# snayfach/MicrobeCensus

Hardware: AMD Instinct MI355X
Metric: reads/sec searched vs marker DB + AGS abs-error, 150 bp @ 1/2/4/8 GPU (higher is better)
Workload: dtype u8/int32

## Files before the change

microbecensus_amd/csrc/k_gapped.h:

```cpp
#pragma once
#include "mc_hip_common.h"

struct McFlankOut { int16_t gain, c1, c2, ident, steps, runs, gapcols, over; };

struct McFlank { int qoff, doff, st, n1, n2; };
__device__ __forceinline__ bool mc_flank_of(const McGapTask &g, int qlen, int dlen, int side, McFlank &f)
{
    if (side == 0) {
        const int qend = g.qfwd + g.qp + g.L, dend = g.qfwd + g.dp + g.L;
        f.qoff = qend; f.doff = dend; f.st = 1; f.n1 = qlen - qend; f.n2 = dlen - dend;
    } else {
        const int qleft = g.qp - g.qbwd, dleft = g.dp - g.qbwd;
        f.qoff = qleft - 1; f.doff = dleft - 1; f.st = -1; f.n1 = qleft; f.n2 = dleft;
    }
    return f.n1 > 2 && f.n2 > 2;
}

__device__ __forceinline__ bool mc_gap_same_segment(const McGapTask &a, const McGapTask &b)
{
    return a.read == b.read && a.sidx == b.sidx && (a.chrono >> 25) == (b.chrono >> 25) && a.qp - a.qbwd == b.qp - b.qbwd && a.dp - a.qbwd == b.dp - b.qbwd &&
           a.qp + a.L + a.qfwd == b.qp + b.L + b.qfwd;
}

__device__ __forceinline__ uint32_t mc_block_alloc_n(uint32_t *counter, uint32_t n)
{
    __shared__ uint32_t wcnt[4], wbase[4];
    const int lane = mc_lane(), wv = threadIdx.x >> 6;
    uint32_t incl = n;
    for (int d = 1; d < 64; d <<= 1) { const uint32_t y = __shfl_up(incl, d); if (lane >= d) incl += y; }
    if (lane == 63) wcnt[wv] = incl;
    __syncthreads();
    if (threadIdx.x == 0) {
        const uint32_t c0 = wcnt[0], c1 = wcnt[1], c2 = wcnt[2], c3 = wcnt[3], tot = c0 + c1 + c2 + c3;
        const uint32_t b = tot ? atomicAdd(counter, tot) : 0u;
        wbase[0] = b; wbase[1] = b + c0; wbase[2] = b + c0 + c1; wbase[3] = b + c0 + c1 + c2;
    }
    __syncthreads();
    const uint32_t r = wbase[wv] + incl - n;
    __syncthreads();
    return r;
}

__global__ void __launch_bounds__(256) k_gap_dedupe(McIndex X, int L, const McGapTask *__restrict__ gaps, uint32_t ngaps, unsigned long long *tab, uint32_t mask, uint32_t *leader,
                                                    uint32_t *key, uint32_t *item, uint32_t *counters)
{
    const uint32_t p = blockIdx.x * 256 + threadIdx.x;
    uint32_t n = 0;
    McFlank fr, fl;
    bool hr = false, hl = false;
    if (p < ngaps && gaps[p].read == MC_TASK_NONE) leader[p] = p;
    else if (p < ngaps) {
        const McGapTask g = gaps[p];
        unsigned long long h = ((unsigned long long)g.read << 32) ^ ((unsigned long long)g.sidx << 12) ^ (unsigned long long)(g.chrono >> 25);
        h ^= ((unsigned long long)(uint16_t)(g.qp - g.qbwd) << 48) ^ ((unsigned long long)(uint16_t)(g.dp - g.qbwd) << 20) ^ ((unsigned long long)(uint16_t)(g.qp + g.L + g.qfwd) << 3);
        h *= 0x9E3779B97F4A7C15ull; h ^= h >> 29; h *= 0xBF58476D1CE4E5B9ull; h ^= h >> 32;
        const unsigned long long mine = (h & ~0x7FFFFFFull) | (unsigned long long)(p + 1);
        uint32_t slot = (uint32_t)h & mask, who = p;
        bool lead = false;
        for (;;) {
            unsigned long long e = tab[slot];
            if (e == 0) e = atomicCAS(&tab[slot], 0ull, mine);
            if (e == 0) { lead = true; break; }
            if ((e & ~0x7FFFFFFull) == (mine & ~0x7FFFFFFull)) {
                const uint32_t q = (uint32_t)(e & 0x7FFFFFFull) - 1;
                if (mc_gap_same_segment(g, gaps[q])) { who = q; break; }
            }
            slot = (slot + 1) & mask;
        }
        leader[p] = who;
        if (lead) {
            const int frame = (int)(g.chrono >> 25), qlen = (L - frame % 3) / 3, dlen = (int)(X.off[g.sidx + 1] - X.off[g.sidx]);
            hr = mc_flank_of(g, qlen, dlen, 0, fr); hl = mc_flank_of(g, qlen, dlen, 1, fl);
            n = (hr ? 1u : 0u) + (hl ? 1u : 0u);
        }
    }
    uint32_t o = mc_block_alloc_n(&counters[C_ITEMS], n);
    if (hr) { key[o] = 1u + (uint32_t)fr.n1; item[o] = 2 * p; o++; }
    if (hl) { key[o] = 1u + (uint32_t)fl.n1; item[o] = 2 * p + 1; }
}

#define MC_GS_BINS 1024u
__global__ void __launch_bounds__(256) k_gap_sort_hist(const uint32_t *__restrict__ key, const uint32_t *__restrict__ n_p, uint32_t cap, uint32_t *hist)
{
    __shared__ uint32_t h[MC_GS_BINS];
    const uint32_t n = *n_p <= cap ? *n_p : 0u;
    for (uint32_t b = threadIdx.x; b < MC_GS_BINS; b += 256) h[b] = 0;
    __syncthreads();
    const uint32_t per = (n + gridDim.x - 1) / gridDim.x, lo = blockIdx.x * per, hi = lo + per < n ? lo + per : n;
    for (uint32_t i = lo + threadIdx.x; i < hi; i += 256) atomicAdd(&h[key[i] & (MC_GS_BINS - 1)], 1u);
    __syncthreads();
    for (uint32_t b = threadIdx.x; b < MC_GS_BINS; b += 256) if (h[b]) atomicAdd(&hist[b], h[b]);
}
__global__ void __launch_bounds__(1024) k_gap_sort_scan(uint32_t *hist)
{
    __shared__ uint32_t s[MC_GS_BINS];
    const uint32_t t = threadIdx.x, v = hist[MC_GS_BINS - 1 - t];
    s[t] = v;
    __syncthreads();
    for (uint32_t d = 1; d < MC_GS_BINS; d <<= 1) { const uint32_t y = t >= d ? s[t - d] : 0u; __syncthreads(); s[t] += y; __syncthreads(); }
    hist[MC_GS_BINS - 1 - t] = s[t] - v;
}
__global__ void __launch_bounds__(256) k_gap_sort_scatter(const uint32_t *__restrict__ key, const uint32_t *__restrict__ item, const uint32_t *__restrict__ n_p, uint32_t cap, uint32_t *base, uint32_t *out)
{
    __shared__ uint32_t h[MC_GS_BINS], at[MC_GS_BINS];
    const uint32_t n = *n_p <= cap ? *n_p : 0u;
    for (uint32_t b = threadIdx.x; b < MC_GS_BINS; b += 256) h[b] = 0;
    __syncthreads();
    const uint32_t per = (n + gridDim.x - 1) / gridDim.x, lo = blockIdx.x * per, hi = lo + per < n ? lo + per : n;
    for (uint32_t i = lo + threadIdx.x; i < hi; i += 256) atomicAdd(&h[key[i] & (MC_GS_BINS - 1)], 1u);
    __syncthreads();
    for (uint32_t b = threadIdx.x; b < MC_GS_BINS; b += 256) { const uint32_t c = h[b]; if (c) at[b] = atomicAdd(&base[b], c); h[b] = 0; }
    __syncthreads();
    for (uint32_t i = lo + threadIdx.x; i < hi; i += 256) { const uint32_t b = key[i] & (MC_GS_BINS - 1); out[at[b] + atomicAdd(&h[b], 1u)] = item[i]; }
}

__global__ void __launch_bounds__(256) k_gap_emit(const McTables *__restrict__ T, McIndex X, int L, const McGapTask *__restrict__ gaps, uint32_t ngaps, const uint32_t *__restrict__ leader,
                                                  const McFlankOut *__restrict__ fout, McHsp *hsps, uint32_t cap_hsps, uint32_t *counters, const McClassPars *__restrict__ P,
                                                  const int32_t *__restrict__ fam, uint8_t *cand, uint64_t *hkeys, uint8_t *low, uint64_t *hplace)
{
    const uint32_t p = blockIdx.x * 256 + threadIdx.x;
    bool keep = false;
    McHsp h;
    if (p < ngaps && gaps[p].read != MC_TASK_NONE) {
        const McGapTask g = gaps[p];
        const uint32_t ld = leader[p];
        const int frame = (int)(g.chrono >> 25), qlen = (L - frame % 3) / 3, dlen = (int)(X.off[g.sidx + 1] - X.off[g.sidx]);
        int score = g.score, nmatch = g.nmatch, qfwd = g.qfwd, dfwd = g.qfwd, qbwd = g.qbwd, dbwd = g.qbwd, alnlen = g.qfwd + g.L + g.qbwd, gapopens = 0, gaptotal = 0;
        McFlank f;
        if (mc_flank_of(g, qlen, dlen, 0, f)) {
            const McFlankOut R = fout[2 * (size_t)ld];
            if (R.gain > 0) { score += R.gain; nmatch += R.ident; qfwd += R.c1; dfwd += R.c2; alnlen += R.steps; gapopens += R.runs; gaptotal += R.gapcols; }
        }
        if (mc_flank_of(g, qlen, dlen, 1, f)) {
            const McFlankOut R = fout[2 * (size_t)ld + 1];
            if (R.gain > 0) { score += R.gain; nmatch += R.ident; qbwd += R.c1; dbwd += R.c2; alnlen += R.steps; gapopens += R.runs; gaptotal += R.gapcols; }
        }
        h.read = g.read; h.chrono = g.chrono;
        keep = mc_make_hsp(*T, L, frame, g, qfwd, dfwd, qbwd, dbwd, score, nmatch, alnlen, gapopens, gaptotal, &h);
        if (keep && cand && mc_hsp_can_classify(*T, *P, X, fam, h)) cand[h.read] = 1;
        if (keep && h.loge < T->loge_thr) low[h.read] = 1;
    }
    const uint32_t o = mc_block_alloc(&counters[C_HSPS], keep);
    if (keep) { if (o < cap_hsps) { hsps[o] = h; hkeys[o] = MC_HSP_KEY(h); hplace[o] = MC_HSP_PLACE(h); } else counters[C_OVERFLOW] = 2; }
}

#define MC_GAP_W 1200
#ifndef MC_GAP_WIN
#define MC_GAP_WIN 36
#endif
#ifndef MC_GAP_WIN2
#define MC_GAP_WIN2 64
#endif
static_assert(MC_GAP_WIN >= 16 && MC_GAP_WIN <= MC_GAP_WIN2, "row 0 of a flank has jEnd + 1 = 16 columns (xdrop_gapped 26.98: mc_gap_begin), and the second window is no narrower than the first");
#define MC_GAP_LANES2 64

__device__ __forceinline__ McFlankOut mc_flank_out(const McGapResult &R)
{
    McFlankOut o;
    o.gain = (int16_t)R.gain; o.c1 = (int16_t)R.c1; o.c2 = (int16_t)R.c2; o.ident = (int16_t)R.ident; o.steps = (int16_t)R.steps; o.runs = (int16_t)R.runs;
    o.gapcols = (int16_t)R.gapcols; o.over = (int16_t)R.overflow;
    return o;
}

__global__ void __launch_bounds__(128) k_gapped(const McTables *__restrict__ T, McIndex X, const uint8_t *__restrict__ frames, int FP, int L,
                                                const McGapTask *__restrict__ gaps, const uint32_t *__restrict__ list, const uint32_t *__restrict__ nitems_p, McFlankOut *fout,
                                                uint32_t *counters, McGapCell *ws, int cap)
{
    __shared__ McHot hot;
    const uint32_t nitems = *nitems_p;
    if (nitems == 0) return;
    mc_load_hot(&hot, T);
    __syncthreads();
    const uint32_t tid = blockIdx.x * blockDim.x + threadIdx.x, nthreads = gridDim.x * blockDim.x;
    McGapCell *C = ws + (size_t)tid * cap;
    for (uint32_t k0 = tid; k0 < nitems; k0 += nthreads) {
        const uint32_t it = list[k0];
        const McGapTask g = gaps[it >> 1];
        const int frame = (int)(g.chrono >> 25), qlen = (L - frame % 3) / 3;
        const uint32_t o0 = X.off[g.sidx];
        McFlank f;
        (void)mc_flank_of(g, qlen, (int)(X.off[g.sidx + 1] - o0), (int)(it & 1), f);
        const McGapResult R = mc_align_gapped(hot, frames + ((int64_t)g.read * 6 + frame) * FP + f.qoff, f.st, X.res + o0 + f.doff, f.st, f.n1, f.n2, C, cap);
        if (R.overflow) counters[C_OVERFLOW] = 5;
        fout[it] = mc_flank_out(R);
    }
}

#define MC_GAP_REFILL 8
template <int W>
struct McGapLds {
    uint2 *cell;
    uint32_t ovf;
    __device__ __forceinline__ void load(int c, int &H, int &D, uint32_t &PH, uint32_t &PD) const
    {
        const uint2 w = cell[c * 64];
        mc_gap_unpack(w.x, w.y, H, D, PH, PD);
    }
    __device__ __forceinline__ void store(int c, int H, int D, uint32_t PH, uint32_t PD)
    {
        uint2 w;
        ovf |= mc_gap_pack(H, D, PH, PD, w.x, w.y);
        cell[c * 64] = w;
    }
    __device__ __forceinline__ int loadH(int c) const { return (int)(cell[c * 64].x << 20) >> 20; }
};

template <int W, int LANES, int REFILL>
__global__ void __launch_bounds__(64) k_gapped_lds(const McTables *__restrict__ T, McIndex X, const uint8_t *__restrict__ frames, int FP, int L,
                                                   const McGapTask *__restrict__ gaps, const uint32_t *__restrict__ list, const uint32_t *__restrict__ nitems_p, McFlankOut *fout,
                                                   uint32_t *retry_count, uint32_t *retry, uint32_t *take)
{
    static_assert(REFILL >= 1 && REFILL <= LANES, "a refill is at most the lanes that take items");
    __shared__ McHot hot;
    __shared__ uint2 win[W * 64];
    const uint32_t nitems = *nitems_p;
    if (nitems == 0) return;
    mc_load_hot(&hot, T);
    __syncthreads();
    const int lane = threadIdx.x;
    McGapLds<W> ws; ws.cell = win + lane; ws.ovf = 0;
    const bool mine = lane < LANES;
    const uint32_t G = gridDim.x, w0 = blockIdx.x;
    constexpr uint32_t WS = (uint32_t)LANES;
    uint32_t wpos = w0 * WS < nitems ? w0 * WS : nitems, wend = wpos + WS < nitems ? wpos + WS : nitems;
    uint32_t pend = 0;
    bool asked = false, dry = false;
    const unsigned long long lt = (1ull << lane) - 1;
    bool active = false;
// ... 73 lines not shown
```

microbecensus_amd/csrc/mc_hip.hip:

```cpp
#include "mc_hip_common.h"
#include "k_translate_seg.h"
#include "k_enumerate.h"
#include "k_eval_seeds.h"
#include "k_gapped.h"
#include "k_order.h"
#include "k_finish.h"
#include "k_grid.h"
#include "k_simulate.h"
#include "k_community.h"
#include "k_varlen.h"
#include "k_classes.h"
#include "k_bootstrap.h"
#include "k_wfit.h"
#include "k_abundance.h"
#include "k_coverage.h"
#include "mc_pieces.h"
#include "mc_owned.h"

#include <map>

struct McCtx {
    McStream stream; hipStream_t side = nullptr, side2 = nullptr;
    McEvent ev[8], ev_fork, ev_join, ev_join2;
    int64_t cap_reads = 0; int pool_len = 0;
    uint32_t cap_tasks = 0, cap_gaps = 0, cap_hsps = 0, cap_rows = 0;
    McDev<uint8_t> d_frames_base; uint8_t *d_frames = nullptr;
    McDev<unsigned long long> d_stats;
    McDev<McSeedTask> d_tasks; McDev<McGapTask> d_gaps; McDev<McHsp> d_hsps, d_v, d_tmp;
    McDev<uint64_t> d_k64, d_hkeys, d_hplace, d_places; McDev<uint32_t> d_idx, d_idxo, d_heads, d_scan, d_gsz, d_nv, d_ghist;
    McDev<uint32_t> d_counters;
    McDev<McRow> d_rows; McDev<uint32_t> d_nrow, d_rowoff; McDev<McBestHit> d_best, d_bestof; McDev<uint8_t> d_low, d_cand;
    McDev<McGapCell> d_gws_full; McDev<uint32_t> d_retry, d_retry2; int gap_threads_full = 0;
    McDev<unsigned long long> d_gtab; uint32_t gtab_slots = 0; McDev<uint32_t> d_gleader; McDev<McFlankOut> d_fout;
    McPin<uint32_t> h_c; McPin<unsigned long long> h_stats; McPin<McBestHit> h_best; size_t h_best_cap = 0;
    const uint8_t *reads = nullptr; int64_t n = 0, first_read_id = 0;
    uint32_t ntasks = 0, ngaps = 0, gpad = 0, nh = 0, nh_all = 0, nheads = 0, nrows = 0, nbest = 0, nsegs = 0;
    bool busy = false;
};

struct mc_handle {
    McHostIndex H;
    std::vector<int32_t> fam;
    int nfam = 0, device = 0;
    McDev<uint8_t> d_res_base; uint8_t *d_res = nullptr; McDev<uint32_t> d_off, d_bstart, d_post; McDev<unsigned long long> d_post8; McDev<uint16_t> d_keys; McDev<int32_t> d_fam;
    McDev<McTables> d_T; McDev<McClassPars> d_P;
    McTables hT; McClassPars hP;
    int read_len = 0, FP = 0; bool run_set = false;
    McDev<uint32_t> d_bitmap;
    McDev<McBucketRec> d_rec;
    McDev<uint32_t> d_filt, d_wild, d_pair; McDev<uint64_t> d_segtab; McDev<unsigned long long> d_rt;
    bool fast_enum = false;
    bool count_traffic = false;
    int pipe_nout = 0;
    bool keep_rows = true;
    bool best_only = false;
    bool rows_stay = false;
    float train_ms[3] = {0, 0, 0};
    float comm_ms[2] = {0, 0};
    int64_t train_bases = 0;
    float boot_ms = 0;
    float wfit_ms = 0;
    bool abund = false; McAbundPars abund_pars = {}; McDev<unsigned long long> d_abund; int64_t abund_searched = 0; float abund_ms = 0;
    McEvent ev_abund[2];
    bool cov = false; McDev<uint32_t> d_cov; McDev<unsigned long long> d_covout; float cov_ms = 0;
    McEvent ev_cov[2];
    McPin<uint8_t> stage_pin[2]; McDev<uint8_t> stage_dev[2]; size_t stage_bytes = 0; McStream copy_stream;
    int64_t nreads = 0, cap_own = 0;
    McDev<uint8_t> d_reads;
    const uint8_t *reads_dev = nullptr;
    McCtx ctx;
    McPin<mc_row> pin_slot[2]; size_t pin_slot_cap[2] = {0, 0}; int pin_cur = 0;
    McStream side, side2;
    McStream rows_stream; McEvent ev_rows; bool rows_pending = false, rows_ever = false;
    std::vector<mc_row> all_rows, split_rows;
    const mc_row *res_rows = nullptr; int64_t n_res_rows = 0;
    std::vector<mc_best_hit> best; mc_stats stats;
    McCtx *best_from = nullptr; uint32_t best_count = 0;
    std::map<int, McTables> vl_tables; double vl_thr = 0;
    McClasses cls = {}; bool cls_set = false, cls_results = false; std::vector<McClassPars> cls_pars;
    std::vector<uint8_t> best_cls; int64_t cls_reads[MC_CL_BINS] = {};
};

static McIndex dev_index(const mc_handle *h)
{
    McIndex X; X.res = h->d_res; X.off = h->d_off; X.bstart = h->d_bstart; X.post = h->d_post; X.post8 = h->d_post8; X.keys = h->d_keys; X.rec = h->d_rec; X.filt = h->d_filt; X.wild = h->d_wild; X.pair = h->d_pair; X.rt = h->d_rt; X.rt_mask = h->H.rt_mask; X.nseq = h->H.nseq;
    return X;
}

extern "C" void mc_debug_live(int64_t out[4]) { for (int k = 0; k < MC_LIVE_N; k++) out[k] = mc_live[k].load(); }

extern "C" int mc_device_count(void)
{
    int n = 0;
    if (hipGetDeviceCount(&n) != hipSuccess) return 0;
    return n;
}

extern "C" void mc_close(mc_handle *h)
{
    if (!h) return;
    (void)hipSetDevice(h->device);
    if (h->rows_stream) (void)hipStreamSynchronize(h->rows_stream);
    delete h;
}

struct McUploader {
    static constexpr size_t CH = (size_t)8 << 20;
    McPin<uint8_t> pin[2]; McEvent ev[2]; McStream st; int k = 0; bool used[2] = {false, false};
    int init()
    {
        if (st.create()) return -1;
        for (int i = 0; i < 2; i++) if (pin[i].alloc(CH) || ev[i].create(false)) return -1;
        return 0;
    }
    int put(void *dst, const void *src, size_t bytes)
    {
        for (size_t at = 0; at < bytes; at += CH) {
            const size_t n = std::min(CH, bytes - at);
            if (used[k]) HIPCK(hipEventSynchronize(ev[k]));
            memcpy(pin[k], (const uint8_t *)src + at, n);
            HIPCK(hipMemcpyAsync((uint8_t *)dst + at, pin[k], n, hipMemcpyHostToDevice, st));
            HIPCK(hipEventRecord(ev[k], st)); used[k] = true;
            k ^= 1;
        }
        return 0;
    }
    int finish() { if (st) HIPCK(hipStreamSynchronize(st)); return 0; }
    ~McUploader() { if (st) (void)hipStreamSynchronize(st); }
};

static int open_impl(mc_handle *h, const int32_t *marker_family, int32_t nfam, int32_t device)
{
    int ndev = 0;
    double t0 = mc_now();
    if (hipGetDeviceCount(&ndev) != hipSuccess || ndev <= 0) { g_err = "no HIP device available: libmcensus_hip has no CPU fallback"; return -1; }
    if (device < 0 || device >= ndev) { g_err = "device index out of range"; return -1; }
    if (nfam > 32) { g_err = "at most 32 gene families are supported"; return -1; }
    const int nseq = h->H.nseq;
    if (nseq > 32767) { g_err = "more than 32767 markers: the HSP sort key (read<<43 | subject<<28 | hit order) holds 15 bits of subject index"; return -1; }
    for (int s = 0; s < nseq; s++) if ((int)(h->H.off[s + 1] - h->H.off[s]) > MC_GAP_W - 8) { g_err = "marker longer than the gapped-extension workspace"; return -1; }
    if (marker_family) h->fam.assign(marker_family, marker_family + nseq); else h->fam.assign((size_t)nseq, 0);
    h->nfam = nfam; h->device = device;
    HIPCK(hipSetDevice(device));
    HIPCK(hipFree(nullptr));
    MC_OT("  HIP runtime, device", t0);
    if (h->side.create() || h->side2.create()) return -1;
    {
        McCtx &c = h->ctx;
        if (c.stream.create()) return -1;
        c.side = h->side; c.side2 = h->side2;
        for (auto &e : c.ev) if (e.create()) return -1;
        if (c.ev_fork.create(false) || c.ev_join.create(false) || c.ev_join2.create(false)) return -1;
        if (c.d_counters.alloc(C_N) || c.d_stats.alloc(S_N) || c.d_ghist.alloc((size_t)MC_GS_BINS)) return -1;
        if (c.h_c.alloc(C_N) || c.h_stats.alloc(S_N)) return -1;
    }
    if (h->rows_stream.create() || h->ev_rows.create(false)) return -1;
    const McHostIndex &H = h->H;
    if (H.res.size() >= MC_TASK_ABS_LIMIT) { g_err = "marker database too large: more than 16 M residues (MC_TASK_W3)"; return -1; }
    if (h->d_res_base.alloc(H.res.size() + 128) || h->d_off.alloc(H.off.size()) || h->d_bstart.alloc(H.bstart.size()) || h->d_post.alloc(H.post.size() + 1) || h->d_post8.alloc((H.post.size() + 1) * MC_POST_WORDS) ||
        h->d_keys.alloc(H.keys.size()) || h->d_fam.alloc((size_t)nseq) || h->d_T.alloc(1) || h->d_P.alloc(1)) return -1;
    HIPCK(hipMemset(h->d_res_base, MC_INV, H.res.size() + 128));
    h->d_res = h->d_res_base + 64;
    if (h->d_bitmap.alloc(H.bitmap.size()) || h->d_filt.alloc(H.filt.size()) || h->d_wild.alloc(H.wild.size()) || h->d_pair.alloc(H.pair.size()) || h->d_rt.alloc(H.rt.size())) return -1;
    if (!H.rec.empty() && h->d_rec.alloc(H.rec.size())) return -1;
    {
        McUploader up;
        if (up.init() || up.put(h->d_res, H.res.data(), H.res.size()) || up.put(h->d_off, H.off.data(), H.off.size() * 4) || up.put(h->d_bstart, H.bstart.data(), H.bstart.size() * 4) ||
            up.put(h->d_post, H.post.data(), H.post.size() * 4) || up.put(h->d_keys, H.keys.data(), H.keys.size() * 2) || up.put(h->d_fam, h->fam.data(), (size_t)nseq * 4) ||
            up.put(h->d_bitmap, H.bitmap.data(), H.bitmap.size() * 4) || up.put(h->d_pair, H.pair.data(), H.pair.size() * 4) || up.put(h->d_wild, H.wild.data(), H.wild.size() * 4) ||
            up.put(h->d_rt, H.rt.data(), H.rt.size() * 8) || up.put(h->d_filt, H.filt.data(), H.filt.size() * 4) ||
            (!H.rec.empty() && up.put(h->d_rec, H.rec.data(), H.rec.size() * sizeof(McBucketRec))) || up.finish()) return -1;
    }
    if (H.nseq > 32767) { g_err = "marker database too large: more than 32,767 sequences (MC_POST8)"; return -1; }
    k_post8<<<dim3((unsigned)((H.post.size() + 255) / 256)), dim3(256)>>>(h->d_post, h->d_off, h->d_res, (uint32_t)H.post.size(), h->d_post8);
    HIPCK(hipDeviceSynchronize());
    MC_OT("  index upload", t0);
    if (H.max_bucket > 2047) { g_err = "a seed bucket holds more than 2047 postings: the hit-order key cannot index it"; return -1; }
    h->fast_enum = (H.freq_thr == 0) && !H.rec.empty() && !getenv("MC_FORCE_SEQUENTIAL_ENUM");
    for (int g = 0; g < 10; g++) if (!(H.letter_p[g] > 0.0)) h->fast_enum = false;
    return 0;
}

static std::mutex g_ixc_mu;
static std::string g_ixc_dir;
extern "C" int mc_set_index_cache(const char *dir)
{
// ... 202 lines not shown
    if (nreads) HIPCK(hipMemcpyAsync(h->d_reads, reads, (size_t)nreads * h->read_len, hipMemcpyHostToDevice, h->ctx.stream));
    HIPCK(hipStreamSynchronize(h->ctx.stream));
    h->reads_dev = h->d_reads; h->nreads = nreads;
    return 0;
}

extern "C" int mc_attach(mc_handle *h, const void *device_reads, int64_t nreads)
{
    if (!h || !h->run_set) { g_err = "mc_set_run() must be called first"; return -1; }
    h->reads_dev = (const uint8_t *)device_reads; h->nreads = nreads;
    return 0;
}

static float ev_ms(hipEvent_t a, hipEvent_t b) { float ms = 0; (void)hipEventElapsedTime(&ms, a, b); return ms; }

static int stage_wait(McCtx &c) { HIPCK(hipStreamSynchronize(c.stream)); return 0; }
static int counters_to_host(McCtx &c) { HIPCK(hipMemcpyAsync(c.h_c, c.d_counters, sizeof(uint32_t) * C_N, hipMemcpyDeviceToHost, c.stream)); return 0; }

#ifdef MC_EXP_TIMING
static int exp_timing_dump(McCtx &c, char stage)
{
    if (stage == 'a') {
        HIPCK(hipStreamSynchronize(c.stream));
        unsigned long long acc[12], cnt[12];
        HIPCK(hipMemcpyFromSymbol(acc, HIP_SYMBOL(g_ts_acc), sizeof acc)); HIPCK(hipMemcpyFromSymbol(cnt, HIP_SYMBOL(g_ts_cnt), sizeof cnt));
        const char *nm[12] = {"flags", "advance", "numbering", "class-0 rounds", "class-1 rounds", "reduction", "owners", "mask", "staging", "translation", "write-out", ""};
        const double waves = (double)((c.n + MC_TS_READS - 1) / MC_TS_READS) * MC_TS_WAVES;
        for (int k = 0; k < 11; k++) fprintf(stderr, "ts-timing %-15s %9.1f cycles/wave  %8.2f entries/wave  total %8.1f Mcycles\n", nm[k], (double)acc[k] / waves, (double)cnt[k] / waves, acc[k] / 1e6);
        unsigned long long z[12] = {0, 0, 0, 0, 0, 0, 0, 0, 0, 0, 0, 0};
        HIPCK(hipMemcpyToSymbol(HIP_SYMBOL(g_ts_acc), z, sizeof z)); HIPCK(hipMemcpyToSymbol(HIP_SYMBOL(g_ts_cnt), z, sizeof z));
    } else {
        HIPCK(hipStreamSynchronize(c.stream)); HIPCK(hipStreamSynchronize(c.side));
        unsigned long long acc[8], cnt[8];
        HIPCK(hipMemcpyFromSymbol(acc, HIP_SYMBOL(g_fh_acc), sizeof acc)); HIPCK(hipMemcpyFromSymbol(cnt, HIP_SYMBOL(g_fh_cnt), sizeof cnt));
        {
            unsigned long long fr[8];
            HIPCK(hipMemcpyFromSymbol(fr, HIP_SYMBOL(g_fr_acc), sizeof fr));
            const char *fn[7] = {"groups", "items", "std::sort", "threshold, keys", "heap sort", "rows", "classification"};
            for (int k = 0; k < 7; k++) fprintf(stderr, "fr-timing %-17s total %9.1f Mcycles (thread wall time, summed)\n", fn[k], fr[k] / 1e6);
            unsigned long long z8[8] = {0, 0, 0, 0, 0, 0, 0, 0};
            HIPCK(hipMemcpyToSymbol(HIP_SYMBOL(g_fr_acc), z8, sizeof z8));
            HIPCK(hipMemcpyFromSymbol(fr, HIP_SYMBOL(g_fr_acc2), sizeof fr));
            const char *gn[8] = {"-", "sort by frame", "sort by start, stable", "choice", "sum statistics", "copies", "groups (count)", "groups linked (count)"};
            for (int k = 1; k < 8; k++) fprintf(stderr, "fg-timing %-22s %12.1f M\n", gn[k], fr[k] / 1e6);
            HIPCK(hipMemcpyToSymbol(HIP_SYMBOL(g_fr_acc2), z8, sizeof z8));
        }
        {
            unsigned long long ev[8];
            HIPCK(hipMemcpyFromSymbol(ev, HIP_SYMBOL(g_ev_acc), sizeof ev));
            const char *en[7] = {"loop, records asked", "survivors queued", "X-drop extension", "HSP, marks", "records written", "residue wait + seed", "growth, gate"};
            for (int k = 0; k < 7; k++) fprintf(stderr, "ev-timing %-21s total %9.1f Mcycles (lane 0 of every wave)\n", en[k], ev[k] / 1e6);
            unsigned long long z8[8] = {0, 0, 0, 0, 0, 0, 0, 0};
            HIPCK(hipMemcpyToSymbol(HIP_SYMBOL(g_ev_acc), z8, sizeof z8));
            unsigned long long tr[4];
            HIPCK(hipMemcpyFromSymbol(tr, HIP_SYMBOL(g_ev_turns), sizeof tr));
            fprintf(stderr, "ev-turns forward: %.1f M lane-turns in %.2f M wave-turns = %.1f lanes of 64; backward: %.1f M in %.2f M = %.1f lanes\n", tr[0] / 1e6, tr[1] / 1e6, tr[1] ? (double)tr[0] / (double)tr[1] : 0.0,
                    tr[2] / 1e6, tr[3] / 1e6, tr[3] ? (double)tr[2] / (double)tr[3] : 0.0);
            HIPCK(hipMemcpyToSymbol(HIP_SYMBOL(g_ev_turns), z8, sizeof tr));
        }
        const char *nm[8] = {"group starts", "groups", "scan, items", "sort", "threshold, ranks", "heap sort", "rows", "other"};
        for (int k = 0; k < 8; k++) fprintf(stderr, "fh-timing %-17s total %9.1f Mcycles %9llu entries\n", nm[k], acc[k] / 1e6, cnt[k]);
        {
            unsigned long long w[12];
            HIPCK(hipMemcpyFromSymbol(w, HIP_SYMBOL(g_fh_worst), sizeof w));
            fprintf(stderr, "fh-worst read: %llu stacked HSPs, %.3f Mcycles:", w[0] & 0xFFFFF, (double)(w[0] >> 20) / 1e6);
            for (int k = 0; k < 8; k++) fprintf(stderr, " %s %.3f", nm[k], (double)w[1 + k] / 1e6);
            fprintf(stderr, "\n");
            unsigned long long z12[12] = {0, 0, 0, 0, 0, 0, 0, 0, 0, 0, 0, 0};
            HIPCK(hipMemcpyToSymbol(HIP_SYMBOL(g_fh_worst), z12, sizeof z12));
        }
        unsigned long long z[8] = {0, 0, 0, 0, 0, 0, 0, 0};
        HIPCK(hipMemcpyToSymbol(HIP_SYMBOL(g_fh_acc), z, sizeof z)); HIPCK(hipMemcpyToSymbol(HIP_SYMBOL(g_fh_cnt), z, sizeof z));
    }
    return 0;
}
#else
static int exp_timing_dump(McCtx &, char) { return 0; }
#endif

static int stage_a(mc_handle *h, McCtx &c)
{
    const int64_t n = c.n;
    const int L = h->read_len, FP = h->FP;
    hipStream_t st = c.stream;
    McIndex X = dev_index(h);
    c.ntasks = c.ngaps = c.gpad = c.nh = c.nheads = c.nrows = c.nbest = c.nsegs = 0;
    HIPCK(hipMemsetAsync(c.d_counters, 0, sizeof(uint32_t) * C_N, st));
    HIPCK(hipMemsetAsync(c.d_stats, 0, sizeof(unsigned long long) * S_N, st));
    if (h->best_only) HIPCK(hipMemsetAsync(c.d_cand, 0, (size_t)n, st));
    HIPCK(hipMemsetAsync(c.d_low, 0, (size_t)n, st));
    HIPCK(hipEventRecord(c.ev[0], st));
    const int64_t threads = n * 6;
    const size_t lds_rest = (size_t)MC_TS_NLNF(FP) * 8 + (size_t)MC_TS_THREADS * MC_TS_STRIDE(FP);
    const size_t lds_staged = (size_t)MC_TS_STAGE(L) + lds_rest, lds_direct = (size_t)MC_TS_STAGE(0) + lds_rest;
    static const int ts_force = getenv("MC_TS_STAGED") ? atoi(getenv("MC_TS_STAGED")) : -1;
    const size_t cu_lds = 160 * 1024 - 1024;
    const bool staged = ts_force >= 0 ? ts_force != 0 : cu_lds / lds_staged >= cu_lds / lds_direct;
    const size_t lds = staged ? lds_staged : lds_direct;
    const unsigned ts_blocks = (unsigned)((n + MC_TS_READS - 1) / MC_TS_READS);
    if (staged) {
        if (lds > 48 * 1024) HIPCK(hipFuncSetAttribute((const void *)k_translate_seg<true>, hipFuncAttributeMaxDynamicSharedMemorySize, (int)lds));
        k_translate_seg<true><<<dim3(ts_blocks), dim3(MC_TS_THREADS), lds, st>>>(h->d_T, c.reads, L, n, c.d_frames, FP, h->d_segtab);
    } else {
        if (lds > 48 * 1024) HIPCK(hipFuncSetAttribute((const void *)k_translate_seg<false>, hipFuncAttributeMaxDynamicSharedMemorySize, (int)lds));
        k_translate_seg<false><<<dim3(ts_blocks), dim3(MC_TS_THREADS), lds, st>>>(h->d_T, c.reads, L, n, c.d_frames, FP, h->d_segtab);
    }
    HIPCK(hipEventRecord(c.ev[1], st));
    if (exp_timing_dump(c, 'a')) return -1;
    if (h->fast_enum) {
        const bool enq = !h->count_traffic;
        const size_t per_wave = enq ? MC_ENQ_WAVE_LDS(FP, L) : sizeof(McEnWave) + MC_EN_WAVE_LDS(FP, L);
        int waves = 0, bpc = 1;
        {
            static const int shapes_q[][2] = {{8, 2}, {4, 4}, {16, 1}, {12, 1}, {4, 3}, {8, 1}, {4, 2}, {4, 1}};
            static const int shapes_c[][2] = {{12, 2}, {8, 3}, {4, 6}, {4, 5}, {16, 1}, {8, 2}, {4, 4}, {12, 1}, {4, 3}, {8, 1}, {4, 2}, {4, 1}};
            if (enq) { for (const auto &sh : shapes_q) if (!waves && (size_t)sh[1] * (64 + sh[0] * per_wave) <= 160 * 1024) { waves = sh[0]; bpc = sh[1]; } }
            else for (const auto &sh : shapes_c) if (!waves && (size_t)sh[1] * (64 + sh[0] * per_wave) <= 160 * 1024) { waves = sh[0]; bpc = sh[1]; }
        }
        if (!waves) { g_err = "reads too long for the seed kernel's LDS layout"; return -1; }
        const size_t lds2 = 64 + waves * per_wave;
#define MC_LAUNCH_EN(KERNEL, WV)                                                                                                                   \
    do {                                                                                                                                           \
        HIPCK(hipFuncSetAttribute((const void *)KERNEL<WV>, hipFuncAttributeMaxDynamicSharedMemorySize, (int)lds2));                               \
        const int blocks_ = (int)std::min<int64_t>((int64_t)256 * bpc, (n + WV - 1) / WV);                                                         \
        KERNEL<WV><<<dim3(blocks_), dim3(64 * WV), lds2, st>>>(h->d_T, X, h->d_bitmap, c.d_frames, FP, L, n, c.d_tasks, c.cap_tasks, c.d_counters, c.d_stats); \
    } while (0)
        if (enq) { if (waves == 16) MC_LAUNCH_EN(k_enumerate_q, 16); else if (waves == 12) MC_LAUNCH_EN(k_enumerate_q, 12); else if (waves == 8) MC_LAUNCH_EN(k_enumerate_q, 8); else MC_LAUNCH_EN(k_enumerate_q, 4); }
        else { if (waves == 16) MC_LAUNCH_EN(k_enumerate_count, 16); else if (waves == 12) MC_LAUNCH_EN(k_enumerate_count, 12); else if (waves == 8) MC_LAUNCH_EN(k_enumerate_count, 8); else MC_LAUNCH_EN(k_enumerate_count, 4); }
#undef MC_LAUNCH_EN
    } else
        k_enumerate<<<dim3((unsigned)((threads + 255) / 256)), dim3(256), 0, st>>>(h->d_T, X, c.d_frames, FP, L, n, c.d_tasks, c.cap_tasks, c.d_counters, c.d_stats);
    HIPCK(hipEventRecord(c.ev[2], st));
    const size_t lds_ev = (size_t)(MC_EV_BS / 64) * MC_EV_QCAP * 32;
    const bool ranges = h->fast_enum && !h->count_traffic;
    HIPCK(hipFuncSetAttribute(ranges ? (const void *)k_eval_seeds<true> : (const void *)k_eval_seeds<false>, hipFuncAttributeMaxDynamicSharedMemorySize, (int)lds_ev));
    if (ranges) k_eval_seeds<true><<<dim3(256u * MC_EV_BPC), dim3(MC_EV_BS), lds_ev, st>>>(h->d_T, X, c.d_frames, FP, L, c.d_tasks, c.d_counters + C_TASKS, c.cap_tasks, c.d_hsps, c.cap_hsps, c.d_gaps, c.cap_gaps, c.d_counters, h->d_P, h->d_fam, h->best_only ? c.d_cand : nullptr, c.d_hkeys, c.d_low, c.d_hplace);
    else k_eval_seeds<false><<<dim3(256u * MC_EV_BPC), dim3(MC_EV_BS), lds_ev, st>>>(h->d_T, X, c.d_frames, FP, L, c.d_tasks, c.d_counters + C_TASKS, c.cap_tasks, c.d_hsps, c.cap_hsps, c.d_gaps, c.cap_gaps, c.d_counters, h->d_P, h->d_fam, h->best_only ? c.d_cand : nullptr, c.d_hkeys, c.d_low, c.d_hplace);
    HIPCK(hipEventRecord(c.ev[3], st));
    return counters_to_host(c);
}

static int stage_b(mc_handle *h, McCtx &c)
{
    const int L = h->read_len, FP = h->FP;
    hipStream_t st = c.stream;
    McIndex X = dev_index(h);
    if (c.h_c[C_OVERFLOW]) { g_err = "seed task / HSP / gap task buffer overflow"; return -2; }
    c.ntasks = c.h_c[C_TASKS];
    const uint32_t ngaps = c.ngaps = c.h_c[C_GAPS];
    c.gpad = c.h_c[C_GPAD];
    if (ngaps) {
        uint32_t slots = 1u << 16;
        while (slots < 2 * ngaps) slots <<= 1;
        if (slots > c.gtab_slots) { if (c.d_gtab.alloc((size_t)slots)) return -1; c.gtab_slots = slots; }
        if (2 * (uint64_t)ngaps > c.cap_hsps) { g_err = "gap task pool larger than the sort buffers"; return -2; }
        uint32_t *gk = (uint32_t *)c.d_k64.get(), *gi = c.d_idx, *gio = c.d_idxo;
        HIPCK(hipMemsetAsync(c.d_gtab, 0, (size_t)slots * 8, st));
        HIPCK(hipMemsetAsync(c.d_ghist, 0, MC_GS_BINS * sizeof(uint32_t), st));
        k_gap_dedupe<<<dim3((ngaps + 255) / 256), dim3(256), 0, st>>>(X, L, c.d_gaps, ngaps, c.d_gtab, slots - 1, c.d_gleader, gk, gi, c.d_counters);
        k_gap_sort_hist<<<dim3(512), dim3(256), 0, st>>>(gk, c.d_counters + C_ITEMS, 2 * ngaps, c.d_ghist);
        k_gap_sort_scan<<<dim3(1), dim3(1024), 0, st>>>(c.d_ghist);
        k_gap_sort_scatter<<<dim3(512), dim3(256), 0, st>>>(gk, gi, c.d_counters + C_ITEMS, 2 * ngaps, c.d_ghist, gio);
        k_gapped_lds<MC_GAP_WIN, 64, MC_GAP_REFILL><<<dim3(std::min<uint32_t>((2 * ngaps + 63) / 64, 256u * 8u)), dim3(64), 0, st>>>(h->d_T, X, c.d_frames, FP, L, c.d_gaps, gio, c.d_counters + C_ITEMS, c.d_fout,
                                                                                                                          c.d_counters + C_RETRY, c.d_retry, c.d_counters + C_GTAKE);
        k_gapped_lds<MC_GAP_WIN2, MC_GAP_LANES2, 1><<<dim3(256u * 4u), dim3(64), 0, st>>>(h->d_T, X, c.d_frames, FP, L, c.d_gaps, c.d_retry, c.d_counters + C_RETRY, c.d_fout, c.d_counters + C_RETRY2, c.d_retry2, c.d_counters + C_GTAKE2);
        k_gapped<<<dim3(c.gap_threads_full / 128), dim3(128), 0, st>>>(h->d_T, X, c.d_frames, FP, L, c.d_gaps, c.d_retry2, c.d_counters + C_RETRY2, c.d_fout, c.d_counters, c.d_gws_full, MC_GAP_W);
        k_gap_emit<<<dim3((ngaps + 255) / 256), dim3(256), 0, st>>>(h->d_T, X, L, c.d_gaps, ngaps, c.d_gleader, c.d_fout, c.d_hsps, c.cap_hsps, c.d_counters, h->d_P, h->d_fam, h->best_only ? c.d_cand : nullptr, c.d_hkeys, c.d_low, c.d_hplace);
    }
    HIPCK(hipEventRecord(c.ev[4], st));
    return counters_to_host(c);
}

static int stage_c(mc_handle *h, McCtx &c)
{
    hipStream_t st = c.stream;
    if (c.h_c[C_OVERFLOW]) { g_err = "HSP buffer overflow"; return -2; }
    const uint32_t nslots = c.h_c[C_HSPS];
    c.nh_all = nslots - c.h_c[C_HPAD];
    c.nh = c.nh_all;
    if (c.nh) {
        const uint32_t n = (uint32_t)c.n;
        const uint8_t *cand = h->best_only ? c.d_cand : nullptr;
        uint32_t *cur = c.d_heads + 1;
        uint64_t *keys = c.d_k64;
        uint32_t *slots = c.d_idxo, *order = c.d_idx, *heavy = c.d_retry2, *heavy2 = c.d_retry2 + c.cap_gaps;
        HIPCK(hipMemsetAsync(c.d_heads, 0, ((size_t)n + 2) * sizeof(uint32_t), st));
        HIPCK(hipMemsetAsync(c.d_nrow, 0, ((size_t)n + 1) * sizeof(uint32_t), st));
        HIPCK(hipMemsetAsync(order, 0xFF, (size_t)nslots * sizeof(uint32_t), st));
        k_bin_count<<<dim3(256u * 8u), dim3(256), 0, st>>>(c.d_hkeys, c.d_counters, c.cap_hsps, cand, cur);
        if (mc_scan_u32(cur, n, cur, c.d_scan, st)) return -1;
        k_bin_scatter<<<dim3(256u * 8u), dim3(256), 0, st>>>(c.d_hkeys, c.d_counters, c.cap_hsps, cand, cur, c.d_hplace, keys, c.d_places, slots);
        uint32_t *heavy3 = heavy2 + c.cap_gaps / 2;
        k_order_lists<<<dim3((n + 255) / 256), dim3(256), 0, st>>>(c.d_heads, n, c.d_counters, heavy, heavy2, heavy3);
        hipStream_t side = c.side, side2 = h->best_only ? c.side : c.side2;
        HIPCK(hipEventRecord(c.ev_fork, st)); HIPCK(hipStreamWaitEvent(c.side, c.ev_fork, 0)); HIPCK(hipStreamWaitEvent(c.side2, c.ev_fork, 0));
        HIPCK(hipFuncSetAttribute((const void *)k_order_heavy<1024, MC_ORDER_LDS>, hipFuncAttributeMaxDynamicSharedMemorySize, (int)(MC_ORDER_LDS * 18)));
        k_order_heavy<1024, MC_ORDER_LDS><<<dim3(256u), dim3(1024), MC_ORDER_LDS * 18, side>>>(keys, c.d_places, slots, c.d_heads, heavy3, c.d_counters + C_ORDER3, c.d_counters + C_OTAKE3, c.d_low, order, c.d_gsz, c.d_nv, c.d_nrow, (uint64_t *)c.d_tmp.get());
        k_order_heavy<256, MC_ORDER_MID><<<dim3(256u * 4u), dim3(256), MC_ORDER_MID * 18, side2>>>(keys, c.d_places, slots, c.d_heads, heavy2, c.d_counters + C_ORDER2, c.d_counters + C_OTAKE2, c.d_low, order, c.d_gsz, c.d_nv, c.d_nrow, (uint64_t *)c.d_tmp.get());
        HIPCK(hipEventRecord(c.ev_join, c.side)); HIPCK(hipEventRecord(c.ev_join2, c.side2));
        k_order_light<<<dim3((n + MC_OL_READS - 1) / MC_OL_READS), dim3(256), 0, st>>>(keys, c.d_places, slots, c.d_heads, n, c.d_low, order, c.d_gsz, c.d_nv, c.d_nrow);
        k_order_heavy<64, MC_ORDER_SMALL><<<dim3(256u * 16u), dim3(64), MC_ORDER_SMALL * 18, st>>>(keys, c.d_places, slots, c.d_heads, heavy, c.d_counters + C_ORDER, c.d_counters + C_OTAKE, c.d_low, order, c.d_gsz, c.d_nv, c.d_nrow, (uint64_t *)c.d_tmp.get());
        HIPCK(hipStreamWaitEvent(st, c.ev_join, 0)); HIPCK(hipStreamWaitEvent(st, c.ev_join2, 0));
        k_order_copy<<<dim3(256u * 8u), dim3(256), 0, st>>>(order, c.d_gsz, c.d_hsps, c.d_heads, n, c.d_v);
    }
    HIPCK(hipEventRecord(c.ev[5], st));
    return 0;
}

static int stage_d(mc_handle *h, McCtx &c)
{
    hipStream_t st = c.stream;
    McIndex X = dev_index(h);
    const uint32_t nh = c.nh, nheads = c.nheads = nh ? (uint32_t)c.n : 0u;
    if (nh) {
        uint32_t *d_heavy = c.d_retry, *d_heavy2 = c.d_retry + c.cap_gaps / 2, *d_heavy3 = c.d_retry + c.cap_gaps;
        uint32_t *d_light = c.d_retry + c.cap_gaps + c.cap_gaps / 2;
        uint32_t *d_heavy1 = c.d_retry2, *d_heap_order = c.d_retry2 + c.cap_gaps;
        const uint32_t light_pitch = (uint32_t)c.cap_reads + 1;
        k_heavy_lists<<<dim3((nheads + 255) / 256), dim3(256), 0, st>>>(c.d_nv, nheads, c.d_nrow, c.d_bestof, c.d_counters, d_heavy, d_light, light_pitch, h->best_only ? MC_FH_MIN_BEST : MC_FH_MIN,
                                                                         d_heavy1, d_heavy2, d_heavy3);
        HIPCK(hipEventRecord(c.ev_fork, st));
        {
            const size_t l1 = (size_t)MC_FH_N1 * 16 + 3 * (size_t)(MC_FH_N1 + 2) * 2, l2 = (size_t)MC_FH_N2 * 16 + 3 * (size_t)(MC_FH_N2 + 2) * 2, l3 = (size_t)MC_FH_N3 * 16 + 3 * (size_t)(MC_FH_N3 + 2) * 2;
            HIPCK(hipFuncSetAttribute((const void *)k_finish_heavy<MC_FH_N3, C_HEAVY3, -1>, hipFuncAttributeMaxDynamicSharedMemorySize, (int)l3));
            HIPCK(hipStreamWaitEvent(c.side, c.ev_fork, 0));
            HIPCK(hipStreamWaitEvent(c.side2, c.ev_fork, 0));
            const unsigned wpc2 = (unsigned)std::min<size_t>(8, std::max<size_t>(1, (size_t)(158 * 1024) / (l2 + 1024)));
            uint32_t *d_sorted1 = c.d_retry2 + c.cap_gaps / 2, *d_sorted2 = c.d_retry2 + c.cap_gaps + c.cap_gaps / 2;
            k_heavy_order<<<dim3(1), dim3(1024), 0, c.side2>>>(d_heavy2, c.d_counters + C_HEAVY2, d_heavy, c.d_nv, 2, d_sorted2);
            k_finish_heavy<MC_FH_N2, C_HEAVY2, -1><<<dim3(256 * wpc2), dim3(64), l2, c.side2>>>(h->d_T, X, h->d_P, h->d_fam, c.d_nv, c.d_heads, nheads, c.d_v, c.d_tmp, c.first_read_id,
                                                                                            c.d_nrow, c.d_bestof, c.d_counters, d_heavy, d_sorted2, nullptr);
            k_finish_heavy<MC_FH_N3, C_HEAVY3, -1><<<dim3(256), dim3(64), l3, c.side2>>>(h->d_T, X, h->d_P, h->d_fam, c.d_nv, c.d_heads, nheads, c.d_v, c.d_tmp, c.first_read_id,
                                                                                         c.d_nrow, c.d_bestof, c.d_counters, d_heavy, d_heavy3, nullptr);
            HIPCK(hipEventRecord(c.ev_join2, c.side2));
            k_heavy_order<<<dim3(1), dim3(1024), 0, c.side>>>(d_heavy1, c.d_counters + C_HEAVY1, d_heavy, c.d_nv, 0, d_sorted1);
            k_finish_heavy<MC_FH_N1, C_HEAVY1, -1><<<dim3(256 * 12), dim3(64), l1, c.side>>>(h->d_T, X, h->d_P, h->d_fam, c.d_nv, c.d_heads, nheads, c.d_v, c.d_tmp, c.first_read_id,
                                                                                            c.d_nrow, c.d_bestof, c.d_counters, d_heavy, d_sorted1, nullptr);
            HIPCK(hipStreamWaitEvent(c.side, c.ev_join2, 0));
            const size_t lh = (size_t)(MC_MAX_M8 + 2) * 64 * 4;
            HIPCK(hipFuncSetAttribute((const void *)k_heap_lanes, hipFuncAttributeMaxDynamicSharedMemorySize, (int)lh));
            k_heap_order<<<dim3(1), dim3(1024), 0, c.side>>>(d_heavy, c.d_nrow, c.d_counters, d_heap_order);
            k_heap_lanes<<<dim3(256), dim3(64), lh, c.side>>>(c.d_heads, nheads, nh, c.d_tmp, c.d_nrow, c.d_counters, d_heavy, d_heap_order);
            k_heavy_rows<<<dim3(256 * 12), dim3(64), 0, c.side>>>(h->d_T, X, h->d_P, h->d_fam, c.d_heads, nheads, c.d_v, c.d_tmp, c.first_read_id, c.d_nrow, c.d_bestof, c.d_counters, d_heavy);
            HIPCK(hipEventRecord(c.ev_join, c.side));
        }
        {
            const size_t lb = 32 * (MC_FH_MIN * 16 + 16), ls = 128 * (16 * 16 + 16);
            HIPCK(hipFuncSetAttribute((const void *)k_finish<32, MC_FH_MIN, 2>, hipFuncAttributeMaxDynamicSharedMemorySize, (int)lb));
            k_finish<32, MC_FH_MIN, 2><<<dim3((nheads + 31) / 32, 2), dim3(32), lb, st>>>(h->d_T, X, h->d_P, h->d_fam, c.d_nv, c.d_heads, nheads, c.d_v, c.d_tmp,
                                                                                 c.first_read_id, c.d_nrow, c.d_bestof, d_light, light_pitch, c.d_counters + C_LIGHT0);
            k_finish<128, 16, 0><<<dim3((nheads + 127) / 128, 2), dim3(128), ls, st>>>(h->d_T, X, h->d_P, h->d_fam, c.d_nv, c.d_heads, nheads, c.d_v, c.d_tmp,
                                                                                     c.first_read_id, c.d_nrow, c.d_bestof, d_light, light_pitch, c.d_counters + C_LIGHT0);
        }
        HIPCK(hipStreamWaitEvent(st, c.ev_join, 0));
        if (mc_scan_u32(c.d_nrow, nheads, c.d_rowoff, c.d_scan, st)) return -1;
        if (h->rows_ever) HIPCK(hipStreamWaitEvent(st, h->ev_rows, 0));
        k_emit_rows<<<dim3((nheads + 255) / 256), dim3(256), 0, st>>>(c.d_heads, nheads, c.d_nrow, c.d_rowoff, c.d_tmp, c.d_rows, c.cap_rows, c.d_bestof, c.d_best, c.d_counters, h->best_only ? 0 : 1);
    }
    HIPCK(hipEventRecord(c.ev[6], st));
    if (exp_timing_dump(c, 'd')) return -1;
    HIPCK(hipMemcpyAsync(c.h_stats, c.d_stats, sizeof(unsigned long long) * S_N, hipMemcpyDeviceToHost, st));
    return counters_to_host(c);
}

static bool rows_stay(const mc_handle *h) { return h->rows_stay || (h->abund && !h->keep_rows); }

static int stage_e(mc_handle *h, McCtx &c)
{
    hipStream_t st = c.stream;
    if (c.nrows && !rows_stay(h)) HIPCK(hipMemcpyAsync(h->pin_slot[h->pin_cur], c.d_rows, sizeof(McRow) * c.nrows, hipMemcpyDeviceToHost, h->rows_stream));
    if (c.nbest) HIPCK(hipMemcpyAsync(c.h_best, c.d_best, sizeof(McBestHit) * c.nbest, hipMemcpyDeviceToHost, st));
    return 0;
}

static void rows_wait(mc_handle *h)
{
    if (h->rows_pending) { (void)hipEventSynchronize(h->ev_rows); h->rows_pending = false; }
}

static void stats_add(mc_stats &tot, const mc_stats &s)
{
    tot.reads += s.reads; tot.seed_tasks += s.seed_tasks; tot.gap_tasks += s.gap_tasks; tot.hsps += s.hsps; tot.rows += s.rows;
    tot.reads_with_rows += s.reads_with_rows; tot.classified += s.classified; tot.bucket_lookups += s.bucket_lookups; tot.key_probes += s.key_probes;
    tot.seed_exact_asks += s.seed_exact_asks; tot.seed_wild_asks += s.seed_wild_asks; tot.seed_pair_asks += s.seed_pair_asks; tot.seed_probes += s.seed_probes;
    tot.ms_translate += s.ms_translate; tot.ms_seed += s.ms_seed; tot.ms_eval += s.ms_eval; tot.ms_gapped += s.ms_gapped;
    tot.ms_sort += s.ms_sort; tot.ms_finish += s.ms_finish; tot.ms_total += s.ms_total;
    tot.range_splits += s.range_splits;
}

static int run_range_once(mc_handle *h, int64_t first, int64_t count, int64_t first_read_id);
static void best_materialize(mc_handle *h);

struct McResults {
    std::vector<mc_row> own_rows, &rows;
    std::vector<mc_best_hit> best; std::vector<uint8_t> tag; mc_stats tot;
    bool want_rows, tagged;
    McResults(bool want_rows_, std::vector<mc_row> *rows_ = nullptr, bool tagged_ = false) : rows(rows_ ? *rows_ : own_rows), want_rows(want_rows_), tagged(tagged_) { memset(&tot, 0, sizeof tot); }
    McResults(const McResults &) = delete;
    void take(mc_handle *h, int tag_ = 0)
    {
        if (want_rows) { rows_wait(h); rows.insert(rows.end(), h->res_rows, h->res_rows + h->n_res_rows); }
        best_materialize(h);
        best.insert(best.end(), h->best.begin(), h->best.end());
        if (tagged) tag.insert(tag.end(), h->best.size(), (uint8_t)tag_);
        stats_add(tot, h->stats);
    }
};

extern "C" int mc_run_range(mc_handle *h, int64_t first, int64_t count, int64_t first_read_id)
{
    if (h && h->pipe_nout) { g_err = "mc_run_range: ranges begun with mc_range_begin() are still in flight"; return -1; }
    int rc = run_range_once(h, first, count, first_read_id);
// ... 1571 lines not shown
```

Before: 64.41 million.

## Add block-local LDS dedupe and epoch-tagged gap hash table to skip per-batch memset

Gap-task dedupe now runs in two levels. First, a 512-slot LDS hash within each 256-thread block collapses duplicate segments. Only block-local leaders then probe the global hash table, which cuts global CAS traffic and random gap reloads. The global table entries also carry an 8-bit epoch, so the per-batch memset of the whole table is replaced by a clear only once every 255 batches; entries from older epochs are treated as empty slots. This adds shared-memory use and two barriers per block, and leader resolution now goes through an LDS indirection.

```diff
diff --git a/microbecensus_amd/csrc/k_gapped.h b/microbecensus_amd/csrc/k_gapped.h
--- a/microbecensus_amd/csrc/k_gapped.h
+++ b/microbecensus_amd/csrc/k_gapped.h
@@ -41,39 +41,78 @@
     return r;
 }
 
-__global__ void __launch_bounds__(256) k_gap_dedupe(McIndex X, int L, const McGapTask *__restrict__ gaps, uint32_t ngaps, unsigned long long *tab, uint32_t mask, uint32_t *leader,
+#define MC_GD_LSLOTS 512u
+#define MC_GD_IDX 0x7FFFFFFull
+#define MC_GD_EPOCH_SHIFT 27
+#define MC_GD_EPOCHS 255u
+#define MC_GD_TAG (~0ull << 35)
+__global__ void __launch_bounds__(256) k_gap_dedupe(McIndex X, int L, const McGapTask *__restrict__ gaps, uint32_t ngaps, unsigned long long *tab, uint32_t mask, uint32_t epoch, uint32_t *leader,
                                                     uint32_t *key, uint32_t *item, uint32_t *counters)
 {
-    const uint32_t p = blockIdx.x * 256 + threadIdx.x;
+    __shared__ McGapTask lg[256];
+    __shared__ unsigned long long ltab[MC_GD_LSLOTS];
+    __shared__ uint32_t lwho[256];
+    const uint32_t t = threadIdx.x, p = blockIdx.x * 256 + t;
     uint32_t n = 0;
     McFlank fr, fl;
     bool hr = false, hl = false;
-    if (p < ngaps && gaps[p].read == MC_TASK_NONE) leader[p] = p;
-    else if (p < ngaps) {
-        const McGapTask g = gaps[p];
-        unsigned long long h = ((unsigned long long)g.read << 32) ^ ((unsigned long long)g.sidx << 12) ^ (unsigned long long)(g.chrono >> 25);
+    for (uint32_t s = t; s < MC_GD_LSLOTS; s += 256) ltab[s] = 0;
+    McGapTask g;
+    g.read = MC_TASK_NONE;
+    if (p < ngaps) { g = gaps[p]; lg[t] = g; }
+    const bool valid = g.read != MC_TASK_NONE;
+    unsigned long long h = 0;
+    if (valid) {
+        h = ((unsigned long long)g.read << 32) ^ ((unsigned long long)g.sidx << 12) ^ (unsigned long long)(g.chrono >> 25);
         h ^= ((unsigned long long)(uint16_t)(g.qp - g.qbwd) << 48) ^ ((unsigned long long)(uint16_t)(g.dp - g.qbwd) << 20) ^ ((unsigned long long)(uint16_t)(g.qp + g.L + g.qfwd) << 3);
         h *= 0x9E3779B97F4A7C15ull; h ^= h >> 29; h *= 0xBF58476D1CE4E5B9ull; h ^= h >> 32;
-        const unsigned long long mine = (h & ~0x7FFFFFFull) | (unsigned long long)(p + 1);
-        uint32_t slot = (uint32_t)h & mask, who = p;
+    }
+    __syncthreads();
+    uint32_t ll = t;
+    if (valid) {
+        const unsigned long long lmine = (h & ~0x1FFull) | 0x100ull | t;
+        uint32_t ls = (uint32_t)(h >> 40) & (MC_GD_LSLOTS - 1);
+        for (;;) {
+            unsigned long long e = ltab[ls];
+            if (e == 0) e = atomicCAS(&ltab[ls], 0ull, lmine);
+            if (e == 0) break;
+            if ((e & ~0x1FFull) == (lmine & ~0x1FFull)) {
+                const uint32_t q = (uint32_t)e & 0xFFu;
+                if (mc_gap_same_segment(g, lg[q])) { ll = q; break; }
+            }
+            ls = (ls + 1) & (MC_GD_LSLOTS - 1);
+        }
+    }
+    uint32_t who = p;
+    if (valid && ll == t) {
+        const unsigned long long ep = (unsigned long long)epoch << MC_GD_EPOCH_SHIFT;
+        const unsigned long long mine = (h & MC_GD_TAG) | ep | (unsigned long long)(p + 1);
+        uint32_t slot = (uint32_t)h & mask;
         bool lead = false;
+        unsigned long long e = tab[slot];
         for (;;) {
-            unsigned long long e = tab[slot];
-            if (e == 0) e = atomicCAS(&tab[slot], 0ull, mine);
-            if (e == 0) { lead = true; break; }
-            if ((e & ~0x7FFFFFFull) == (mine & ~0x7FFFFFFull)) {
-                const uint32_t q = (uint32_t)(e & 0x7FFFFFFull) - 1;
+            if ((e & (0xFFull << MC_GD_EPOCH_SHIFT)) != ep) {
+                const unsigned long long seen = atomicCAS(&tab[slot], e, mine);
+                if (seen == e) { lead = true; break; }
+                e = seen;
+                continue;
+            }
+            if ((e & MC_GD_TAG) == (mine & MC_GD_TAG)) {
+                const uint32_t q = (uint32_t)(e & MC_GD_IDX) - 1;
                 if (mc_gap_same_segment(g, gaps[q])) { who = q; break; }
             }
             slot = (slot + 1) & mask;
-        }
-        leader[p] = who;
+            e = tab[slot];
+        }
         if (lead) {
             const int frame = (int)(g.chrono >> 25), qlen = (L - frame % 3) / 3, dlen = (int)(X.off[g.sidx + 1] - X.off[g.sidx]);
             hr = mc_flank_of(g, qlen, dlen, 0, fr); hl = mc_flank_of(g, qlen, dlen, 1, fl);
             n = (hr ? 1u : 0u) + (hl ? 1u : 0u);
         }
     }
+    lwho[t] = who;
+    __syncthreads();
+    if (p < ngaps) leader[p] = lwho[ll];
     uint32_t o = mc_block_alloc_n(&counters[C_ITEMS], n);
     if (hr) { key[o] = 1u + (uint32_t)fr.n1; item[o] = 2 * p; o++; }
     if (hl) { key[o] = 1u + (uint32_t)fl.n1; item[o] = 2 * p + 1; }
diff --git a/microbecensus_amd/csrc/mc_hip.hip b/microbecensus_amd/csrc/mc_hip.hip
--- a/microbecensus_amd/csrc/mc_hip.hip
+++ b/microbecensus_amd/csrc/mc_hip.hip
@@ -31,7 +31,8 @@
     McDev<uint32_t> d_counters;
     McDev<McRow> d_rows; McDev<uint32_t> d_nrow, d_rowoff; McDev<McBestHit> d_best, d_bestof; McDev<uint8_t> d_low, d_cand;
     McDev<McGapCell> d_gws_full; McDev<uint32_t> d_retry, d_retry2; int gap_threads_full = 0;
-    McDev<unsigned long long> d_gtab; uint32_t gtab_slots = 0; McDev<uint32_t> d_gleader; McDev<McFlankOut> d_fout;
+    McDev<unsigned long long> d_gtab; uint32_t gtab_slots = 0, gtab_epoch = 0; McDev<uint32_t> d_gleader;
+    McDev<McFlankOut> d_fout;
     McPin<uint32_t> h_c; McPin<unsigned long long> h_stats; McPin<McBestHit> h_best; size_t h_best_cap = 0;
     const uint8_t *reads = nullptr; int64_t n = 0, first_read_id = 0;
     uint32_t ntasks = 0, ngaps = 0, gpad = 0, nh = 0, nh_all = 0, nheads = 0, nrows = 0, nbest = 0, nsegs = 0;
@@ -540,12 +541,13 @@
     if (ngaps) {
         uint32_t slots = 1u << 16;
         while (slots < 2 * ngaps) slots <<= 1;
-        if (slots > c.gtab_slots) { if (c.d_gtab.alloc((size_t)slots)) return -1; c.gtab_slots = slots; }
+        if (slots > c.gtab_slots) { if (c.d_gtab.alloc((size_t)slots)) return -1; c.gtab_slots = slots; c.gtab_epoch = MC_GD_EPOCHS; }
+        if (c.gtab_epoch >= MC_GD_EPOCHS) { HIPCK(hipMemsetAsync(c.d_gtab, 0, (size_t)c.gtab_slots * 8, st)); c.gtab_epoch = 0; }
+        c.gtab_epoch++;
         if (2 * (uint64_t)ngaps > c.cap_hsps) { g_err = "gap task pool larger than the sort buffers"; return -2; }
         uint32_t *gk = (uint32_t *)c.d_k64.get(), *gi = c.d_idx, *gio = c.d_idxo;
-        HIPCK(hipMemsetAsync(c.d_gtab, 0, (size_t)slots * 8, st));
         HIPCK(hipMemsetAsync(c.d_ghist, 0, MC_GS_BINS * sizeof(uint32_t), st));
-        k_gap_dedupe<<<dim3((ngaps + 255) / 256), dim3(256), 0, st>>>(X, L, c.d_gaps, ngaps, c.d_gtab, slots - 1, c.d_gleader, gk, gi, c.d_counters);
+        k_gap_dedupe<<<dim3((ngaps + 255) / 256), dim3(256), 0, st>>>(X, L, c.d_gaps, ngaps, c.d_gtab, slots - 1, c.gtab_epoch, c.d_gleader, gk, gi, c.d_counters);
         k_gap_sort_hist<<<dim3(512), dim3(256), 0, st>>>(gk, c.d_counters + C_ITEMS, 2 * ngaps, c.d_ghist);
         k_gap_sort_scan<<<dim3(1), dim3(1024), 0, st>>>(c.d_ghist);
         k_gap_sort_scatter<<<dim3(512), dim3(256), 0, st>>>(gk, gi, c.d_counters + C_ITEMS, 2 * ngaps, c.d_ghist, gio);
```

After: 64.38 million. About the same (-0.0%).
